# mfouda/epsilon

Hardware: AMD Instinct MI355X
Metric: ADMM iters/sec, dense Lasso 1e4x5e4 (higher is better)
Workload: dtype f32

## Files before the change

### epsilon_amd/csrc/kernels_fused.hip

```cpp
#include <hip/hip_runtime.h>

#include <cstdlib>
#include <type_traits>

#include "kernels.h"
#include "kernels_fused_chain.h"

namespace eps {
namespace k {

namespace {

constexpr int kBlock = 256;

template <class T, int NR, int BS, int MODE>
__global__ __launch_bounds__(BS, 2) void LassoFusedStreamKernelT(
    int64_t m, int64_t n, const T* __restrict__ A, int64_t lda, const T* __restrict__ w,
    FusedScalarsT<T> c, T* u, T* x0, T* x1, T* y0, T* y1, T* y1prev, T* __restrict__ tpart,
    unsigned* epoch, T* e0, T* e1) {
  typedef typename Chunk<T>::V V;
  constexpr int R = Chunk<T>::R;
  __shared__ T red[2][BS / 64];
  if (epoch != nullptr && blockIdx.x == 0 && threadIdx.x == 0) *epoch += 1u;
  const int tid = threadIdx.x, lane = tid & 63, wave = tid >> 6;
  const V zero = T(0);
  V wv[NR], tp[NR];
  int64_t row[NR];
#pragma unroll
  for (int q = 0; q < NR; ++q) {
    row[q] = (static_cast<int64_t>(q) * BS + tid) * R;
    wv[q] = row[q] < m ? *reinterpret_cast<const V*>(w + row[q]) : zero;
    tp[q] = zero;
  }
  const int64_t npairs = (n + 1) / 2;
  auto column = [&](int64_t step) -> int64_t {
    const int64_t jp = blockIdx.x + (step >> 1) * gridDim.x;
    const int64_t j = 2 * jp + (step & 1);
    return (jp < npairs && j < n) ? j : -1;
  };
  auto load = [&](V (&a)[NR], int64_t j) {
    const T* cp = A + j * lda;
#pragma unroll
    for (int q = 0; q < NR; ++q) {
      if (row[q] < m) a[q] = __builtin_nontemporal_load(reinterpret_cast<const V*>(cp + row[q]));
      else a[q] = zero;
    }
  };
  V cur[NR], nxt[NR];
  int64_t step = 0;
  int64_t j = column(0);
  if (j >= 0) load(cur, j);
  int par = 0;
  while (j >= 0) {
    int64_t jn = column(step + 1);
    if (jn < 0 && ((step + 1) & 1)) jn = column(step + 2);
    const int64_t step_n = (jn >= 0 && column(step + 1) < 0) ? step + 2 : step + 1;
    if (jn >= 0) load(nxt, jn);
    const T uj = u[j], y0j = y0[j], y1j = y1[j];
    T u1j = T(0);
    if (MODE == 1) u1j = e0[j];
    T d = T(0);
#pragma unroll
    for (int q = 0; q < NR; ++q)
#pragma unroll
      for (int r = 0; r < R; ++r) d += cur[q][r] * wv[q][r];
    d = WaveSumT<T>(d);
    if (lane == 0) red[par][wave] = d;
    __syncthreads();
    d = red[par][0];
#pragma unroll
    for (int w2 = 1; w2 < BS / 64; ++w2) d += red[par][w2];
    par ^= 1;
    FusedScalarsT<T> cj = c;
    if (c.alpha_v != nullptr) cj.alpha = c.alpha_v[j];
    if (c.beta_v != nullptr) cj.beta = c.beta_v[j];
    T v0n;
    if (MODE == 0) {
      T nx0, nx1, ny0, ny1, nu;
      v0n = ChainOneT<T>(d, cj, uj, y0j, y1j, &nx0, &nx1, &ny0, &ny1, &nu);
      if (tid == 0) {
        y1prev[j] = y1j;
        x0[j] = nx0;
        x1[j] = nx1;
        y0[j] = ny0;
        y1[j] = ny1;
        u[j] = nu;
      }
    } else {
      T nx0, nx1, nz0, nz1, nu0, nu1;
      v0n = ChainTwoBlockT<T>(d, cj, y0j, y1j, uj, u1j, &nx0, &nx1, &nz0, &nz1, &nu0, &nu1);
      if (tid == 0) {
        y1prev[j] = y0j;
        e1[j] = y1j;
        x0[j] = nx0;
        x1[j] = nx1;
        y0[j] = nz0;
        y1[j] = nz1;
        u[j] = nu0;
        e0[j] = nu1;
      }
    }
#pragma unroll
    for (int q = 0; q < NR; ++q)
#pragma unroll
      for (int r = 0; r < R; ++r) tp[q][r] += cur[q][r] * v0n;
#pragma unroll
    for (int q = 0; q < NR; ++q) cur[q] = nxt[q];
    j = jn;
    step = step_n;
  }
  T* out = tpart + static_cast<int64_t>(blockIdx.x) * m;
#pragma unroll
  for (int q = 0; q < NR; ++q)
    if (row[q] < m) *reinterpret_cast<V*>(out + row[q]) = tp[q];
}

template <class T, int NR, int BS>
void LaunchFused(const LassoFusedArgs& a, int grid) {
  const LassoBatchInst<T> i = Narrow<T>(a.inst);
  T* e0 = a.chain == 1 ? a.e0.as<T>() : nullptr;
  T* e1 = a.chain == 1 ? a.e1.as<T>() : nullptr;
  hipLaunchKernelGGL(
      (a.chain == 1 ? LassoFusedStreamKernelT<T, NR, BS, 1> : LassoFusedStreamKernelT<T, NR, BS, 0>),
      dim3(grid), dim3(BS), 0, Runtime::Get().stream(), a.m, a.n, a.A.as<T>(), a.lda, i.w,
      ScalarsOf<T>(i, a.a0, a.inst.a1), i.u, i.x0, i.x1, i.y0, i.y1, i.y1prev, i.tpart, a.epoch, e0, e1);
}

template <class T>
void LaunchFusedT(const LassoFusedArgs& a, int grid, int block) {
  const int64_t need = (a.m + Chunk<T>::R * block - 1) / (Chunk<T>::R * block);
  if (block == 256) {
    if (need <= 1) LaunchFused<T, 1, 256>(a, grid);
    else if (need <= 2) LaunchFused<T, 2, 256>(a, grid);
    else if (need <= 4) LaunchFused<T, 4, 256>(a, grid);
    else if (need <= 8) LaunchFused<T, 8, 256>(a, grid);
    else LaunchFused<T, 10, 256>(a, grid);
    return;
  }
  if constexpr (std::is_same<T, float>::value) {
    if (need <= 2) return LaunchFused<T, 2, 512>(a, grid);
    if (need <= 5) return LaunchFused<T, 5, 512>(a, grid);
  }
  if (need <= 8) LaunchFused<T, 8, 512>(a, grid);
  else LaunchFused<T, 10, 512>(a, grid);
}

}

namespace {

constexpr int kNormBlocks = 64;

template <class T>
__global__ __launch_bounds__(kBlock) void LassoFusedNormsKernel(
    int64_t n, const T* __restrict__ u, const T* __restrict__ y0, const T* __restrict__ y1,
    const T* __restrict__ y1prev, double* partial, unsigned* ticket, double* out,
    const unsigned* peer_err) {
  __shared__ double red[kBlock / 64][5];
  __shared__ bool last;
  const int64_t per = (n + gridDim.x - 1) / gridDim.x;
  const int64_t lo = blockIdx.x * per;
  int64_t hi = lo + per;
  if (hi > n) hi = n;
  double s[5] = {0, 0, 0, 0, 0};
  for (int64_t i = lo + threadIdx.x; i < hi; i += kBlock) {
    const double a = y0[i], b = y1[i], c = y1prev[i], d = u[i];
    s[0] += a * a;
    s[1] += b * b;
    s[2] += (a + b) * (a + b);
    s[3] += (b - c) * (b - c);
    s[4] += d * d;
  }
  const int lane = threadIdx.x & 63, wave = threadIdx.x >> 6;
#pragma unroll
  for (int k = 0; k < 5; ++k) {
    const double t = WaveSumT<double>(s[k]);
    if (lane == 0) red[wave][k] = t;
  }
  __syncthreads();
  if (threadIdx.x < 5) {
    const int k = threadIdx.x;
    const double t = ((red[0][k] + red[1][k]) + red[2][k]) + red[3][k];
    __hip_atomic_store(partial + blockIdx.x * 5 + k, t, __ATOMIC_RELAXED, __HIP_MEMORY_SCOPE_AGENT);
  }
  asm volatile("s_waitcnt vmcnt(0)" ::: "memory");
  __syncthreads();
  if (threadIdx.x == 0) {
    const unsigned prev = __hip_atomic_fetch_add(ticket, 1u, __ATOMIC_RELAXED, __HIP_MEMORY_SCOPE_AGENT);
    last = prev == gridDim.x - 1;
  }
  __syncthreads();
  if (!last) return;
  if (threadIdx.x < 5) {
    const int k = threadIdx.x;
    double t = 0;
    for (unsigned b = 0; b < gridDim.x; ++b)
      t += __hip_atomic_load(partial + b * 5 + k, __ATOMIC_RELAXED, __HIP_MEMORY_SCOPE_AGENT);
    out[k] = t;
  }
  if (threadIdx.x == 5)
    out[5] = (peer_err != nullptr &&
              __hip_atomic_load(peer_err, __ATOMIC_RELAXED, __HIP_MEMORY_SCOPE_AGENT) != 0u) ? 1.0 : 0.0;
  if (threadIdx.x == 0) __hip_atomic_store(ticket, 0u, __ATOMIC_RELAXED, __HIP_MEMORY_SCOPE_AGENT);
}

}

void LassoFusedNorms(const DVec& u, const DVec& y0, const DVec& y1, const DVec& y1prev, double* out6,
                     const DVec& work, const unsigned* peer_err) {
  const int64_t n = u.n;
  EPS_CHECK(y0.n == n && y1.n == n && y1prev.n == n && y0.dt == u.dt && y1.dt == u.dt && y1prev.dt == u.dt);
  EPS_CHECK(work.dt == F64 && work.n >= kNormBlocks * 5 + 1);
  int64_t grid = (n + 4 * kBlock - 1) / (4 * kBlock);
  if (grid > kNormBlocks) grid = kNormBlocks;
  if (grid < 1) grid = 1;
  double* partial = work.as<double>();
  unsigned* ticket = reinterpret_cast<unsigned*>(partial + kNormBlocks * 5);
  ProfScope prof("lasso_fused_norms", n);
  if (u.dt == F32)
    hipLaunchKernelGGL(LassoFusedNormsKernel<float>, dim3(static_cast<unsigned>(grid)), dim3(kBlock), 0,
                       Runtime::Get().stream(), n, u.as<float>(), y0.as<float>(), y1.as<float>(),
                       y1prev.as<float>(), partial, ticket, out6, peer_err);
  else
    hipLaunchKernelGGL(LassoFusedNormsKernel<double>, dim3(static_cast<unsigned>(grid)), dim3(kBlock), 0,
                       Runtime::Get().stream(), n, u.as<double>(), y0.as<double>(), y1.as<double>(),
                       y1prev.as<double>(), partial, ticket, out6, peer_err);
  EPS_HIP(hipGetLastError());
}

bool LassoFusedSupported(int64_t m, int64_t n, const DVec& A, int64_t lda) {
  if (n < 1 || reinterpret_cast<uintptr_t>(A.data()) % 16 != 0) return false;
  if (A.dt == F32) return m >= 4 && m % 4 == 0 && lda % 4 == 0 && m <= 20 * 1024;
  return m >= 2 && m % 2 == 0 && lda % 2 == 0 && m <= 10 * 1024;
}

int LassoFusedBlock(int64_t m, int64_t n, DType dt) {
  (void)n;
  if (dt == F64) return m > 5 * 1024 ? 512 : 256;
  if (m > 10 * 1024) return 512;
  static const char* env = std::getenv("EPSILON_HIP_FUSED_BLOCK");
  if (env && std::atoi(env) == 512 && m >= 2048) return 512;
  return 256;
}

int LassoFusedGrid(int64_t m, int64_t n, DType dt) {
  int64_t npairs = (n + 1) / 2;
  const int64_t rows_per_chunk = dt == F32 ? 4 : 2;
  const bool one_per_cu = LassoFusedBlock(m, n, dt) == 512 && m > 512 * 5 * rows_per_chunk;
  int64_t g = one_per_cu ? 256 : 512;
  static const char* env = std::getenv("EPSILON_HIP_FUSED_GRID");
  if (env && std::atoi(env) > 0) g = std::atoi(env);
  if (g > npairs) g = npairs;
  if (g < 1) g = 1;
  const int64_t per = (npairs + g - 1) / g;
  g = (npairs + per - 1) / per;
  return static_cast<int>(g < 1 ? 1 : g);
}

void LassoFusedPass(const LassoFusedArgs& a) {
  EPS_CHECK(LassoFusedSupported(a.m, a.n, a.A, a.lda));
  const DType dt = a.A.dt;
  const LassoInstance& s = a.inst;
  EPS_CHECK(s.w.n == a.m && s.w.dt == dt);
  for (const DVec* v : {&s.u, &s.x0, &s.x1, &s.y0, &s.y1, &s.y1prev})
    EPS_CHECK(v->n == a.n && v->dt == dt);
  for (const DVec* v : {&s.alpha_vec, &s.beta_vec})
    if (v->n > 0) EPS_CHECK(v->n == a.n && v->dt == dt);
  if (a.chain == 1) EPS_CHECK(a.e0.n == a.n && a.e1.n == a.n && a.e0.dt == dt && a.e1.dt == dt);
  const int grid = LassoFusedGrid(a.m, a.n, dt);
  const int block = LassoFusedBlock(a.m, a.n, dt);
  EPS_CHECK(s.tpart.n >= static_cast<int64_t>(grid) * a.m && s.tpart.dt == dt);
  EPS_CHECK(reinterpret_cast<uintptr_t>(s.w.data()) % 16 == 0 &&
            reinterpret_cast<uintptr_t>(s.tpart.data()) % 16 == 0);
  ProfScope prof("lasso_fused", a.m, a.n);
  if (dt == F32) LaunchFusedT<float>(a, grid, block);
  else LaunchFusedT<double>(a, grid, block);
  EPS_HIP(hipGetLastError());
}

}
}
```

### epsilon_amd/csrc/kernels_fused_chain.h

```cpp
#pragma once

#include <hip/hip_runtime.h>

#include "kernels.h"

namespace eps {
namespace k {
namespace {

template <class T> struct Chunk;
template <> struct Chunk<float> {
  static constexpr int R = 4;
  typedef float V __attribute__((ext_vector_type(4)));
};
template <> struct Chunk<double> {
  static constexpr int R = 2;
  typedef double V __attribute__((ext_vector_type(2)));
};

template <class T> struct FusedScalarsT {
  T kappa;
  T Bs, Cs, a1, lam, alpha, beta, M;
  T a0, inv_aa;
  const T* alpha_v;
  const T* beta_v;
};

template <class T> LassoBatchInst<T> Narrow(const LassoInstance& s) {
  LassoBatchInst<T> d;
  d.w = s.w.as<T>();
  d.tpart = s.tpart.as<T>();
  d.u = s.u.as<T>();
  d.x0 = s.x0.as<T>();
  d.x1 = s.x1.as<T>();
  d.y0 = s.y0.as<T>();
  d.y1 = s.y1.as<T>();
  d.y1prev = s.y1prev.as<T>();
  d.alpha_v = s.alpha_vec.n > 0 ? s.alpha_vec.as<T>() : nullptr;
  d.beta_v = s.beta_vec.n > 0 ? s.beta_vec.as<T>() : nullptr;
  d.p = s.p.as<T>();
  d.rhs = s.rhs.n > 0 ? s.rhs.as<T>() : nullptr;
  d.kappa = static_cast<T>(s.kappa);
  d.pkappa = static_cast<T>(s.pkappa);
  d.Bs = static_cast<T>(s.Bs);
  d.Cs = static_cast<T>(s.Cs);
  d.a1 = static_cast<T>(s.a1);
  d.lam = static_cast<T>(s.lam);
  d.alpha = static_cast<T>(s.alpha);
  d.beta = static_cast<T>(s.beta);
  d.M = static_cast<T>(s.M);
  return d;
}

template <class T> FusedScalarsT<T> ScalarsOf(const LassoBatchInst<T>& i, double a0, double a1) {
  return {i.kappa, i.Bs, i.Cs, i.a1, i.lam, i.alpha, i.beta, i.M,
          static_cast<T>(a0), static_cast<T>(1.0 / (a0 * a0 + a1 * a1)), i.alpha_v, i.beta_v};
}

template <class T> __device__ inline T WaveSumT(T v) {
#pragma unroll
  for (int off = 32; off > 0; off >>= 1) v += __shfl_down(v, off, 64);
  return v;
}

template <class T> __device__ inline T ScaledZoneOneT(T xi, T lam, T alpha, T beta, T M) {
  if (fabs(xi) <= M) return xi;
  if (xi > M + lam * alpha) return xi - lam * alpha;
  if (xi < -M - lam * beta) return xi + lam * beta;
  if (xi > T(0)) return M;
  return -M;
}

template <class T>
__device__ inline T ChainOneT(T d, const FusedScalarsT<T>& c, T u, T y0p, T y1p, T* x0o, T* x1o,
                              T* y0o, T* y1o, T* uo) {
  const T v0 = ((u - y0p) - y1p) + y0p;
  const T x0 = c.kappa * d + v0;
  const T y0 = x0;
  const T u1 = v0 - y0;
  const T u2 = u1 + y1p;
  const T vin = c.Bs * u2;
  const T xz = ScaledZoneOneT<T>(vin, c.lam, c.alpha, c.beta, c.M);
  const T x1 = c.Cs * xz;
  const T y1 = c.a1 * x1;
  const T u3 = u2 - y1;
  *x0o = x0;
  *x1o = x1;
  *y0o = y0;
  *y1o = y1;
  *uo = u3;
  return ((u3 - y0) - y1) + y0;
}

template <class T>
__device__ inline T ChainTwoBlockT(T d, const FusedScalarsT<T>& c, T z0p, T z1p, T u0p, T u1p, T* x0o,
                                   T* x1o, T* z0o, T* z1o, T* u0o, T* u1o) {
  const T v0 = z0p - u0p;
  const T v1 = z1p - u1p;
  const T x0 = c.kappa * d + v0;
  const T x1 = c.Cs * ScaledZoneOneT<T>(c.Bs * v1, c.lam, c.alpha, c.beta, c.M);
  const T w0 = x0 + u0p;
  const T w1 = x1 + u1p;
  const T t = (c.a0 * w0 + c.a1 * w1) * c.inv_aa;
  const T z0 = w0 - c.a0 * t;
  const T z1 = w1 - c.a1 * t;
  const T u0 = u0p + (x0 - z0);
  const T u1 = u1p + (x1 - z1);
  *x0o = x0;
  *x1o = x1;
  *z0o = z0;
  *z1o = z1;
  *u0o = u0;
  *u1o = u1;
  return z0 - u0;
}

}
}
}
```

Measured before the change: 3235.

## Stage per-column ADMM scalars through LDS in batches and double-buffer column loads

Per-column scalar inputs (u, y0, y1, alpha/beta, e0) are now gathered cooperatively into shared memory for 128 steps at a time, and outputs are written back in batches instead of per-column global loads and stores by thread 0. The streaming loop becomes ping-pong buffered with a precomputed step count, clamped unsigned byte offsets plus masking instead of branchy bounded loads, and asm barriers to pin registers. Launch bounds rise to 4 waves/EU for 512-thread blocks with small NR. This aims to remove scalar global-memory latency from the per-column critical path, at the cost of extra syncs, more LDS use, and register pressure.

Result: no change. 3208 (-0.9%).

```diff
diff --git a/epsilon_amd/csrc/kernels_fused.hip b/epsilon_amd/csrc/kernels_fused.hip
--- a/epsilon_amd/csrc/kernels_fused.hip
+++ b/epsilon_amd/csrc/kernels_fused.hip
@@ -14,90 +14,96 @@
 constexpr int kBlock = 256;
 
 template <class T, int NR, int BS, int MODE>
-__global__ __launch_bounds__(BS, 2) void LassoFusedStreamKernelT(
+__global__ __launch_bounds__(BS, (BS == 512 && NR <= 5) ? 4 : 2) void LassoFusedStreamKernelT(
     int64_t m, int64_t n, const T* __restrict__ A, int64_t lda, const T* __restrict__ w,
     FusedScalarsT<T> c, T* u, T* x0, T* x1, T* y0, T* y1, T* y1prev, T* __restrict__ tpart,
     unsigned* epoch, T* e0, T* e1) {
   typedef typename Chunk<T>::V V;
   constexpr int R = Chunk<T>::R;
-  __shared__ T red[2][BS / 64];
+  constexpr int NIN = MODE == 1 ? 6 : 5;
+  constexpr int NOUT = MODE == 1 ? 8 : 6;
+  constexpr int NW = BS / 64;
+  __shared__ T lds[2 * NW + kStageCols * (NIN + NOUT)];
+  T* const red = lds;
+  T* const sin = lds + 2 * NW;
+  T* const sout = sin + kStageCols * NIN;
   if (epoch != nullptr && blockIdx.x == 0 && threadIdx.x == 0) *epoch += 1u;
   const int tid = threadIdx.x, lane = tid & 63, wave = tid >> 6;
   const V zero = T(0);
   V wv[NR], tp[NR];
-  int64_t row[NR];
+  const int trow = tid * R, mi = static_cast<int>(m);
+  unsigned offc[NR];
 #pragma unroll
   for (int q = 0; q < NR; ++q) {
-    row[q] = (static_cast<int64_t>(q) * BS + tid) * R;
-    wv[q] = row[q] < m ? *reinterpret_cast<const V*>(w + row[q]) : zero;
+    const int r = q * BS * R + trow;
+    offc[q] = static_cast<unsigned>(r < mi ? r : mi - R) * static_cast<unsigned>(sizeof(T));
     tp[q] = zero;
   }
+#pragma unroll
+  for (int q = 0; q < NR; ++q)
+    wv[q] = *reinterpret_cast<const V*>(reinterpret_cast<const char*>(w) + offc[q]);
+  MaskColumnT<T, NR, BS>(wv, trow, mi);
+  auto column = [&](int64_t step) -> int64_t { return StepColumn(step, n); };
+  auto load = [&](V (&a)[NR], int64_t j) { LoadColumnT<T, NR>(a, A + j * lda, offc); };
+  const T* const src_mode0[5] = {u, y0, y1, c.alpha_v, c.beta_v};
+  const T* const src_mode1[6] = {u, y0, y1, c.alpha_v, c.beta_v, e0};
+  const T fill[6] = {T(0), T(0), T(0), c.alpha, c.beta, T(0)};
+  T* const dst_mode0[6] = {y1prev, x0, x1, y0, y1, u};
+  T* const dst_mode1[8] = {y1prev, x0, x1, y0, y1, u, e1, e0};
   const int64_t npairs = (n + 1) / 2;
-  auto column = [&](int64_t step) -> int64_t {
-    const int64_t jp = blockIdx.x + (step >> 1) * gridDim.x;
-    const int64_t j = 2 * jp + (step & 1);
-    return (jp < npairs && j < n) ? j : -1;
-  };
-  auto load = [&](V (&a)[NR], int64_t j) {
-    const T* cp = A + j * lda;
-#pragma unroll
-    for (int q = 0; q < NR; ++q) {
-      if (row[q] < m) a[q] = __builtin_nontemporal_load(reinterpret_cast<const V*>(cp + row[q]));
-      else a[q] = zero;
-    }
-  };
-  V cur[NR], nxt[NR];
-  int64_t step = 0;
-  int64_t j = column(0);
-  if (j >= 0) load(cur, j);
+  const int64_t mypairs = (npairs - blockIdx.x + gridDim.x - 1) / gridDim.x;
+  const int64_t nsteps = 2 * mypairs - (column(2 * mypairs - 1) < 0 ? 1 : 0);
+  int64_t step = 0, base = 0;
   int par = 0;
-  while (j >= 0) {
-    int64_t jn = column(step + 1);
-    if (jn < 0 && ((step + 1) & 1)) jn = column(step + 2);
-    const int64_t step_n = (jn >= 0 && column(step + 1) < 0) ? step + 2 : step + 1;
-    if (jn >= 0) load(nxt, jn);
-    const T uj = u[j], y0j = y0[j], y1j = y1[j];
+  auto body = [&](auto has_next, V (&cur)[NR], V (&nxt)[NR]) {
+#pragma unroll
+    for (int q = 0; q < NR; ++q) asm volatile("" : "+v"(cur[q]));
+    if constexpr (decltype(has_next)::value) load(nxt, column(step + 1));
+    MaskColumnT<T, NR, BS>(cur, trow, mi);
+    const T* si = sin + (step - base) * NIN;
+    const T uj = si[0], y0j = si[1], y1j = si[2];
+    FusedScalarsT<T> cj = c;
+    cj.alpha = si[3];
+    cj.beta = si[4];
     T u1j = T(0);
-    if (MODE == 1) u1j = e0[j];
+    if (MODE == 1) u1j = si[NIN - 1];
     T d = T(0);
 #pragma unroll
     for (int q = 0; q < NR; ++q)
 #pragma unroll
       for (int r = 0; r < R; ++r) d += cur[q][r] * wv[q][r];
     d = WaveSumT<T>(d);
-    if (lane == 0) red[par][wave] = d;
+    if (lane == 0) red[par * NW + wave] = d;
     __syncthreads();
-    d = red[par][0];
-#pragma unroll
-    for (int w2 = 1; w2 < BS / 64; ++w2) d += red[par][w2];
+    d = red[par * NW];
+#pragma unroll
+    for (int w2 = 1; w2 < NW; ++w2) d += red[par * NW + w2];
     par ^= 1;
-    FusedScalarsT<T> cj = c;
-    if (c.alpha_v != nullptr) cj.alpha = c.alpha_v[j];
-    if (c.beta_v != nullptr) cj.beta = c.beta_v[j];
+    T* so = sout + (step - base) * NOUT;
     T v0n;
     if (MODE == 0) {
       T nx0, nx1, ny0, ny1, nu;
       v0n = ChainOneT<T>(d, cj, uj, y0j, y1j, &nx0, &nx1, &ny0, &ny1, &nu);
       if (tid == 0) {
-        y1prev[j] = y1j;
-        x0[j] = nx0;
-        x1[j] = nx1;
-        y0[j] = ny0;
-        y1[j] = ny1;
-        u[j] = nu;
+        so[0] = y1j;
+        so[1] = nx0;
+        so[2] = nx1;
+        so[3] = ny0;
+        so[4] = ny1;
+        so[5] = nu;
       }
     } else {
       T nx0, nx1, nz0, nz1, nu0, nu1;
       v0n = ChainTwoBlockT<T>(d, cj, y0j, y1j, uj, u1j, &nx0, &nx1, &nz0, &nz1, &nu0, &nu1);
       if (tid == 0) {
-        y1prev[j] = y0j;
-        e1[j] = y1j;
-        x0[j] = nx0;
-        x1[j] = nx1;
-        y0[j] = nz0;
-        y1[j] = nz1;
-        u[j] = nu0;
-        e0[j] = nu1;
+        so[0] = y0j;
+        so[1] = nx0;
+        so[2] = nx1;
+        so[3] = nz0;
+        so[4] = nz1;
+        so[5] = nu0;
+        so[6] = y1j;
+        so[7] = nu1;
       }
     }
 #pragma unroll
@@ -105,14 +111,38 @@
 #pragma unroll
       for (int r = 0; r < R; ++r) tp[q][r] += cur[q][r] * v0n;
 #pragma unroll
-    for (int q = 0; q < NR; ++q) cur[q] = nxt[q];
-    j = jn;
-    step = step_n;
+    for (int q = 0; q < NR; ++q) asm volatile("" : "+v"(tp[q]));
+    ++step;
+  };
+  V bufa[NR], bufb[NR];
+  load(bufa, column(0));
+  const std::true_type next;
+  const std::false_type none;
+  while (step < nsteps) {
+    if (MODE == 0) StageIn<T, 5, BS>(sin, src_mode0, reinterpret_cast<const T(&)[5]>(fill), base, n);
+    else StageIn<T, 6, BS>(sin, src_mode1, fill, base, n);
+    __syncthreads();
+    const int64_t end = base + kStageCols < nsteps ? base + kStageCols : nsteps;
+    const int64_t lim = end < nsteps ? end : nsteps - 1;
+    while (step + 1 < lim) {
+      body(next, bufa, bufb);
+      body(next, bufb, bufa);
+    }
+    if (step < lim) {
+      body(next, bufa, bufb);
+      body(none, bufb, bufa);
+    } else if (step < end) {
+      body(none, bufa, bufb);
+    }
+    __syncthreads();
+    if (MODE == 0) StageOut<T, 6, BS>(sout, dst_mode0, base, n);
+    else StageOut<T, 8, BS>(sout, dst_mode1, base, n);
+    base += kStageCols;
   }
   T* out = tpart + static_cast<int64_t>(blockIdx.x) * m;
 #pragma unroll
   for (int q = 0; q < NR; ++q)
-    if (row[q] < m) *reinterpret_cast<V*>(out + row[q]) = tp[q];
+    if (trow < mi - q * BS * R) *reinterpret_cast<V*>(reinterpret_cast<char*>(out) + offc[q]) = tp[q];
 }
 
 template <class T, int NR, int BS>
diff --git a/epsilon_amd/csrc/kernels_fused_chain.h b/epsilon_amd/csrc/kernels_fused_chain.h
--- a/epsilon_amd/csrc/kernels_fused_chain.h
+++ b/epsilon_amd/csrc/kernels_fused_chain.h
@@ -63,6 +63,60 @@
   return v;
 }
 
+template <class T, int NR>
+__device__ inline void LoadColumnT(typename Chunk<T>::V (&a)[NR], const T* cp, const unsigned (&offc)[NR]) {
+  typedef typename Chunk<T>::V V;
+#pragma unroll
+  for (int q = 0; q < NR; ++q) {
+    unsigned off = offc[q];
+    asm volatile("" : "+v"(off));
+    a[q] = __builtin_nontemporal_load(reinterpret_cast<const V*>(reinterpret_cast<const char*>(cp) + off));
+  }
+}
+
+template <class T, int NR, int BS>
+__device__ inline void MaskColumnT(typename Chunk<T>::V (&a)[NR], int trow, int m) {
+  typedef typename Chunk<T>::V V;
+  constexpr int R = Chunk<T>::R;
+  const V zero = T(0);
+#pragma unroll
+  for (int q = 0; q < NR; ++q) a[q] = trow < m - q * BS * R ? a[q] : zero;
+}
+
+constexpr int kStageCols = 128;
+
+__device__ inline int64_t StepColumn(int64_t step, int64_t n) {
+  const int64_t jp = blockIdx.x + (step >> 1) * gridDim.x;
+  const int64_t j = 2 * jp + (step & 1);
+  return (jp < (n + 1) / 2 && j < n) ? j : -1;
+}
+
+template <class T, int NF, int BS>
+__device__ inline void StageIn(T* img, const T* const (&src)[NF], const T (&fill)[NF], int64_t base,
+                               int64_t n) {
+  for (int l = threadIdx.x; l < kStageCols; l += BS) {
+    const int64_t j = StepColumn(base + l, n);
+    if (j >= 0) {
+      T v[NF];
+#pragma unroll
+      for (int f = 0; f < NF; ++f) v[f] = (src[f] != nullptr ? src[f] : src[0])[j];
+#pragma unroll
+      for (int f = 0; f < NF; ++f) img[l * NF + f] = src[f] != nullptr ? v[f] : fill[f];
+    }
+  }
+}
+
+template <class T, int NF, int BS>
+__device__ inline void StageOut(const T* img, T* const (&dst)[NF], int64_t base, int64_t n) {
+  for (int l = threadIdx.x; l < kStageCols; l += BS) {
+    const int64_t j = StepColumn(base + l, n);
+    if (j >= 0) {
+#pragma unroll
+      for (int f = 0; f < NF; ++f) dst[f][j] = img[l * NF + f];
+    }
+  }
+}
+
 template <class T> __device__ inline T ScaledZoneOneT(T xi, T lam, T alpha, T beta, T M) {
   if (fabs(xi) <= M) return xi;
   if (xi > M + lam * alpha) return xi - lam * alpha;
```
